# DemianMArin/HMM_Training

Measured on NVIDIA B200. Metric: baum_welch_frames_per_s_per_iter, higher is better.
Workload: dtype f64

## Files before the change

hmm_training_b200/csrc/bw.cu:

```cuda
#include <algorithm>
#include <cstdlib>
#include <functional>
#include <memory>
#include <numeric>

#include "bw_kernels.cuh"
#include "bwltr_kernels.cuh"
#include "viterbi_kernels.cuh"

namespace hmmb {

__global__ void k_load_B(const double *__restrict__ B, int N, int M, double *__restrict__ Bt,
                         int32_t *__restrict__ b_has_zero) {
    const size_t w = blockIdx.y;
    for (int e = blockIdx.x * blockDim.x + threadIdx.x; e < N * M; e += gridDim.x * blockDim.x) {
        const int k = e / N, j = e - k * N;
        const double v = B[(w * N + j) * M + k];
        Bt[w * (size_t)M * N + e] = v > 0.0 ? v : 0.0;
        if (!(v > 0.0) && b_has_zero) b_has_zero[w] = 1;
    }
}
__global__ void k_load_clamped(const double *__restrict__ src, int64_t n, double *__restrict__ dst) {
    for (int64_t e = (int64_t)blockIdx.x * blockDim.x + threadIdx.x; e < n; e += (int64_t)gridDim.x * blockDim.x) {
        const double v = src[e];
// ... 710 lines not shown
        cudaError_t e = cudaMemcpyAsync(&bad, d_bad, sizeof(int), cudaMemcpyDeviceToHost, c.stream);
        if (e == cudaSuccess) e = cudaStreamSynchronize(c.stream);
        if (e != cudaSuccess) rc = cuda_fail(e, "prepare sync", __FILE__, __LINE__);
    }
    dev_free(d_tmp);
    if (rc != HMMB_OK) return rc;
    if (bad) {
        set_error("codeword out of range: some observation is >= M=%d (reference: IndexError)", M);
        return HMMB_ERR_RANGE;
    }
    return HMMB_OK;
}

}

using namespace hmmb;

struct hmmb_bw {
    SeqSet s;
    SeqSet sl;
    bool has_ltr = false;
    bool use_ltr = false;
    uint8_t *d_allfull = nullptr;
    bool check_bad = false;
    std::unique_ptr<PendingPrepare> pend_release;
    void *d_raw = nullptr;
    bool ltr_only = false;
    int raw_idx_bytes = 0;
    uint32_t *d_thinmask = nullptr;
    int32_t *d_thin_new = nullptr;
    int32_t *d_redo = nullptr;
    int32_t *d_redo_in = nullptr;
    int32_t *d_slot_of = nullptr;
    int32_t *act_cur = nullptr;
    int64_t slot_cap = 0, rstride = 0;
    int n_slots = 0;
    int64_t n_thin_total = 0;
    int bpieces = 0, bpieces_issued = 0;
    cudaEvent_t bt_ready[PendingPrepare::MAX_STAGES] = {};
    double *d_ptmp = nullptr;
    std::vector<int64_t> keep_offsets;
    std::vector<int32_t> keep_words;
    SeqSet &cur() { return use_ltr ? sl : s; }
    int W = 0, N = 0, M = 0;
    double *d_pi = nullptr, *d_A = nullptr, *d_Bt = nullptr;
    double *d_spill = nullptr, *d_llseq = nullptr, *d_accum = nullptr, *d_partials = nullptr;
// ... 20 lines not shown
    bool estep_reduced = false;
    bool params_set = false, any_active = true;
};

static double2 *spill4(hmmb_bw *h) { return reinterpret_cast<double2 *>(h->d_spill) + (size_t)BWD4_SPILL_PAD * 64; }

static void bw_drop_pieces(hmmb_bw *h) {
    for (auto &e : h->bt_ready) {
        if (e) event_put(e);
        e = nullptr;
    }
    h->bpieces = h->bpieces_issued = 0;
    dev_free(h->d_ptmp);
    h->d_ptmp = nullptr;
}

static void bw_release(hmmb_bw *h) {
    if (h->d_ptmp && ctx().inited) cudaStreamSynchronize(ctx().copy_stream);
    bw_drop_pieces(h);
    h->pend_release.reset();
    h->s.release();
    h->sl.release();
    dev_free(h->d_allfull);
    dev_free(h->d_raw);
    dev_free(h->d_pi); dev_free(h->d_A); dev_free(h->d_Bt); dev_free(h->d_spill); dev_free(h->d_llseq);
    dev_free(h->d_accum); dev_free(h->d_partials); dev_free(h->d_prev); dev_free(h->d_hist); dev_free(h->d_active);
    dev_free(h->d_iters); dev_free(h->d_any); dev_free(h->d_cta_begin); dev_free(h->d_cta_begin_fine); dev_free(h->d_seq_begin);
    dev_free(h->d_bzero); dev_free(h->d_flag_base); dev_free(h->d_newflags); dev_free(h->d_nexact); dev_free(h->d_exact_scratch);
    dev_free(h->d_thinmask); dev_free(h->d_thin_new); dev_free(h->d_redo); dev_free(h->d_redo_in); dev_free(h->d_slot_of);
}

static int bw_alloc_accum(hmmb_bw *h) {
    dev_free(h->d_accum);
    h->d_accum = nullptr;
    h->accum_n = (int64_t)h->W * h->astride + (int64_t)h->world * h->W * 2 + (int64_t)h->world * h->slot_cap * h->rstride;
    return dev_alloc_t(&h->d_accum, (size_t)h->accum_n);
}

static int bw_set_params_impl(hmmb_bw *h, const double *pi0, const double *A0, const double *B0, bool sync);
static int bw_after_sync(hmmb_bw *h);

static int bw_finish_create(hmmb_bw *h, int64_t R) {
    Ctx &c = ctx();
    SeqSet &s = h->s;
    const int W = h->W, N = h->N, M = h->M;
    h->nacc = (int64_t)N + (int64_t)N * N + (int64_t)M * N;
// ... 22 lines not shown
    TRYF(dev_alloc_t(&h->d_flag_base, (size_t)std::max<int64_t>(R, 1) + FLAG_HDR));
    h->d_flag = h->d_flag_base + FLAG_HDR;
    TRYF(dev_alloc_t(&h->d_newflags, 1));
    TRYF(dev_alloc_t(&h->d_nexact, 1));
    {
        h->exact_stride = (int64_t)std::max(s.tmax_all, 1) * N;
        int64_t warps = std::min<int64_t>((int64_t)c.sm_count * 8, std::max<int64_t>(1, (256LL << 20) / (h->exact_stride * 8)));
        warps = std::min<int64_t>(warps, std::max<int64_t>(1, (R + 31) / 32));
        h->exact_grid = (int)std::max<int64_t>(1, (warps + BW_WARPS - 1) / BW_WARPS);
        TRYF(dev_alloc_t(&h->d_exact_scratch, (size_t)h->exact_grid * BW_WARPS * h->exact_stride));
    }
    TRYF(dev_alloc_t(&h->d_seq_begin, (size_t)W + 1));
    TRYF(h2d_small(h->d_seq_begin, s.seq_begin.data(), (W + 1) * sizeof(int64_t)));
    size_t spill_bytes;
    if (s.special4) {
        spill_bytes = (size_t)(std::max<int64_t>(s.spill_steps, 1) + BWD4_SPILL_PAD) * 64 * sizeof(double2);
        TRYF(dev_alloc_t(&h->d_partials, (size_t)std::max(std::max(s.ncta, s.ncta_fine), 1) * h->pstride));
        TRYF(dev_alloc_t(&h->d_cta_begin, (size_t)W + 1));
        if (s.ncta_fine > 0) {
            TRYF(dev_alloc_t(&h->d_cta_begin_fine, (size_t)W + 1));
            TRYF(h2d_small(h->d_cta_begin_fine, s.cta_begin_fine.data(), (W + 1) * sizeof(int32_t)));
        }
        TRYF(dev_alloc_t(&h->d_allfull, (size_t)std::max<int64_t>(R, 1)));
        TRYF(h2d_small(h->d_cta_begin, s.cta_begin.data(), (W + 1) * sizeof(int32_t)));
    } else {
        spill_bytes = (size_t)std::max<int64_t>(s.frames, 1) * N * sizeof(double);
        if (h->has_ltr) {
            spill_bytes = std::max(spill_bytes, (size_t)std::max<int64_t>(h->sl.spill_steps, 1) * 32 * N * sizeof(double));
            TRYF(dev_alloc_t(&h->d_allfull, (size_t)std::max<int64_t>(R, 1)));
        }
    }
    int rc = dev_alloc((void **)&h->d_spill, spill_bytes);
    if (rc != HMMB_OK) {
        set_error("alpha spill of %.2f GB does not fit in device memory; shard the sequences over more GPUs",
                  spill_bytes / 1e9);
        return HMMB_ERR_OOM;
    }
#undef TRYF
#undef CUDAF
    return HMMB_OK;
}



int hmmb_bw_create(hmmb_bw_t **out, const void *obs, int idx_bytes, int obs_on_device, const int64_t *offsets,
                   const int32_t *word_of_seq, int64_t R, int W, int N, int M) {
// ... 331 lines not shown
    int nw = bidiag ? BWD4_MAX_WARPS : 12;
    auto bytes = [&](int w) { return (size_t)M * rep * 4 * sizeof(double) + (size_t)w * M * 4 * sizeof(double) + (size_t)w * 4 * sizeof(double); };
    const size_t avail = smem_optin > 20 * 1024 ? smem_optin - 20 * 1024 : 0;
    while (nw > 1 && bytes(nw) > avail) --nw;
    *smem = bytes(nw);
    return nw;
}

template <bool BIDIAG, int MT, int REP>
static int launch_special_estep(hmmb_bw *h) {
    Ctx &c = ctx();
    SeqSet &s = h->s;
    if (s.ncta == 0) { s.pend.reset(); return HMMB_OK; }
    const size_t smem_f = (size_t)h->M * 5 * sizeof(double) + (size_t)((h->M + 15) & ~15);
    size_t smem_b = 0;
    const int bwd_threads = 32 * bwd4_warps(h->M, REP, BIDIAG, c.smem_optin, &smem_b);
    HMMB_CUDA(cudaFuncSetAttribute((k_bw_bwd4<BIDIAG, MT, REP>), cudaFuncAttributeMaxDynamicSharedMemorySize, (int)smem_b));
    const CtaWork *stage_work = s.ncta_fine > 0 ? s.d_work_fine : s.d_work;
    const int stage_ncta = s.ncta_fine > 0 ? s.ncta_fine : s.ncta;
    auto launch_range = [&](int c0, int c1) -> int {
        if (c1 <= c0) return HMMB_OK;
        HMMB_LAUNCH("bw_forward", k_bw_fwd4<BIDIAG>, (c1 - c0) * FWD4_SPLIT, BW_THREADS, smem_f, stage_work + c0, s.d_blks, (const uint4 *)s.d_obs,
                    s.d_len, h->d_pi, h->d_A, h->d_Bt, h->M, spill4(h), h->d_llseq, h->act_cur, h->d_flag,
                    h->d_allfull, FWD4_SPLIT, SYM_MASK);
        HMMB_LAUNCH("bw_backward", (k_bw_bwd4<BIDIAG, MT, REP>), c1 - c0, bwd_threads, smem_b, stage_work + c0, s.d_blks, (const uint4 *)s.d_obs,
                    s.d_len, h->d_A, h->d_Bt, h->M, spill4(h), h->d_llseq, h->act_cur, h->d_bzero,
                    h->d_allfull, h->d_partials + (size_t)c0 * h->pstride, h->pstride, h->d_flag, h->d_newflags);
        return HMMB_OK;
    };
    if (s.pend) {
        PendingPrepare &p = *s.pend;
        int bdone = 0, cdone = 0;
        cudaStream_t main_stream = c.stream;
        const bool side = p.nstage > 2;
        struct Restore { Ctx &c; cudaStream_t s; ~Restore() { c.stream = s; } } restore{c, main_stream};
        if (side) {
            cudaEvent_t fork = event_get();
            HMMB_CUDA(cudaEventRecord(fork, main_stream));
            for (auto st : c.stage_stream) HMMB_CUDA(cudaStreamWaitEvent(st, fork, 0));
            event_put(fork);
        }
        for (int j = 0; j < p.nstage; ++j) {
            if (side) c.stream = c.stage_stream[j & 1];
            HMMB_CUDA(cudaStreamWaitEvent(c.stream, p.up->ev[p.ev_index[j]], 0));
            HMMB_TRY(launch_repack_range(s, p.up->d_raw, p.idx_bytes, bdone, p.blk_end[j], s.d_bad));
            HMMB_TRY(launch_range(cdone, p.cta_end[j]));
            bdone = p.blk_end[j];
            cdone = p.cta_end[j];
        }
        c.stream = main_stream;
        if (side) {
            for (auto st : c.stage_stream) {
                cudaEvent_t join = event_get();
                HMMB_CUDA(cudaEventRecord(join, st));
                HMMB_CUDA(cudaStreamWaitEvent(main_stream, join, 0));
                event_put(join);
            }
        }
        h->check_bad = true;
        h->pend_release = std::move(s.pend);
        HMMB_TRY((launch_exact<uint16_t, true>(h)));
        HMMB_LAUNCH("bw_exact", k_bw_llstat_fix, stage_ncta, BW_THREADS, 0, stage_work, s.d_blks, h->d_llseq, h->act_cur,
                    h->d_flag, h->d_partials, h->pstride, h->M);
        h->estep_fine = s.ncta_fine > 0;
        return HMMB_OK;
    }
    h->estep_fine = false;
    HMMB_LAUNCH("bw_forward", k_bw_fwd4<BIDIAG>, (s.ncta_fwd ? s.ncta_fwd : s.ncta) * FWD4_SPLIT, BW_THREADS, smem_f,
                s.ncta_fwd ? s.d_work_fwd : s.d_work, s.d_blks, (const uint4 *)s.d_obs,
                s.d_len, h->d_pi, h->d_A, h->d_Bt, h->M, spill4(h), h->d_llseq, h->act_cur, h->d_flag,
                h->d_allfull, FWD4_SPLIT, SYM_MASK);
    HMMB_TRY((launch_exact<uint16_t, true>(h)));
    HMMB_LAUNCH("bw_backward", (k_bw_bwd4<BIDIAG, MT, REP>), s.ncta, bwd_threads, smem_b, s.d_work, s.d_blks, (const uint4 *)s.d_obs,
                s.d_len, h->d_A, h->d_Bt, h->M, spill4(h), h->d_llseq, h->act_cur, h->d_bzero,
                h->d_allfull, h->d_partials, h->pstride, h->d_flag, h->d_newflags);
    return HMMB_OK;
}

template <int NS>
static int launch_ltr_estep(hmmb_bw *h) {
    SeqSet &s = h->sl;
    if (s.ncta == 0) return HMMB_OK;
    const int M = h->M;
    const size_t smem_f = (size_t)M * NS * 8 + (size_t)M * 8 + (size_t)M * 2;
    const size_t smem_b = (size_t)M * NS * 8 + (size_t)LTR_WARPS * 32 * Ltr<NS>::ROWB + (size_t)2 * NS * 8 +
                          (size_t)LTR_WARPS * 2 * NS * 8;
    HMMB_CUDA(cudaFuncSetAttribute(k_bw_fwdL<NS>, cudaFuncAttributeMaxDynamicSharedMemorySize, (int)smem_f));
    HMMB_CUDA(cudaFuncSetAttribute(k_bw_bwdL<NS>, cudaFuncAttributeMaxDynamicSharedMemorySize, (int)smem_b));
    if (s.pend) {
        Ctx &c = ctx();
        PendingPrepare &p = *s.pend;
        int bdone = 0, cdone = 0;
        cudaStream_t main_stream = c.stream;
        const bool side = p.nstage > 2;
        struct Restore { Ctx &c; cudaStream_t s; ~Restore() { c.stream = s; } } restore{c, main_stream};
        if (side) {
            cudaEvent_t fork = event_get();
            HMMB_CUDA(cudaEventRecord(fork, main_stream));
// ... 618 lines not shown
```

hmm_training_b200/csrc/bw4_kernels.cuh:

```cuda
#pragma once

#include <type_traits>

#include "hmm_device.cuh"

namespace hmmb {

constexpr int BW_THREADS = 128;
constexpr int BW_WARPS = BW_THREADS / 32;
constexpr int SPC4 = 8;
constexpr unsigned SYM_MASK = 0x7ffu;
constexpr int SYM_BITS = 11;
constexpr int BW4_MAX_M = 512;
constexpr int BWD4_MAX_WARPS = 16;
constexpr int FWD4_SPLIT = 4;
constexpr int BWD4_REP = 8;

constexpr int REPACK_WARPS = 8;
__device__ __forceinline__ unsigned lanes_with_my_bit(unsigned sym, int bit) {
    int mine;
    asm("bfe.s32 %0, %1, %2, 1;" : "=r"(mine) : "r"(sym), "r"(bit));
    const unsigned set = __ballot_sync(0xffffffffu, mine != 0);
    return ~(set ^ (unsigned)mine);
}
// ... 92 lines not shown
        for (int j = 0; j < 4; ++j) row[i] |= (__ldg(Aw + i * 4 + j) > 0.0) ? (1u << j) : 0u;
    }
    Masks4 mk;
    mk.lutF = mk.lutB = 0ull;
    for (unsigned m = 0; m < 16; ++m) {
        unsigned f = 0u, b = 0u;
#pragma unroll
        for (int i = 0; i < 4; ++i) {
            if ((m >> i) & 1u) f |= row[i];
            if (row[i] & m) b |= 1u << i;
        }
        mk.lutF |= (unsigned long long)f << (m * 4u);
        mk.lutB |= (unsigned long long)b << (m * 4u);
    }
    mk.pmask = 0u;
    if (piw) {
#pragma unroll
        for (int j = 0; j < 4; ++j) mk.pmask |= (__ldg(piw + j) > 0.0) ? (1u << j) : 0u;
    }
    return mk;
}
__device__ __forceinline__ double tiny_if(unsigned m, int j) { return __hiloint2double(0, (int)((m >> j) & 1u)); }

template <bool BIDIAG, bool SPILL, bool VECB = true, int REP = 1>
__device__ __forceinline__ double fwd4_run(int T, int tmax, const uint4 *__restrict__ op,
                                           const double2 *__restrict__ sB01, const double2 *__restrict__ sB23,
                                           const double *__restrict__ sBmax,
                                           const unsigned char *__restrict__ sBmask, const double *a,
                                           const double (&p)[4], double rmax, const Masks4 &mk,
                                           double2 *__restrict__ sp, bool &allfull, int slot = 0,
                                           unsigned symmask = SYM_MASK) {
    using S16 = Sym<uint16_t>;
    double al0 = 0.0, al1 = 0.0, al2 = 0.0, al3 = 0.0;
    double e0 = 0.0, e1 = 0.0, e2 = 0.0, e3 = 0.0;
    long long esum = 0;
    unsigned m = 0u;
    bool stop = false;
    bool allf = true;
    double ll = neg_inf();
    const double tiny = tiny_pos();
    const int nch = (tmax + SPC4 - 1) / SPC4;
    uint4 wnext = nch > 0 ? __ldg(op) : make_uint4(0, 0, 0, 0);
    for (int c = 0; c < nch; ++c) {
        uint4 w = wnext;
        if (c + 1 < nch) wnext = __ldg(op + (size_t)(c + 1) * 32);
#pragma unroll 2
        for (int s = 0; s < SPC4; ++s) {
            const int t = c * SPC4 + s;
            const unsigned sym = S16::pop_front(w) & symmask;
            if (t < T && !stop) {
                const double2 b01 = sB01[sym * REP + slot], b23 = sB23[sym * REP + slot];
                const unsigned r = (t == 0) ? mk.pmask : lut4(mk.lutF, m);
                m = r & (unsigned)sBmask[sym];
                double n0, n1, n2, n3, at0, at1, at2, at3;
                if (m == 0xFu && t > 0) {
                    if (BIDIAG) {
                        n0 = fma(al0, a[0], tiny);
                        n1 = fma(al1, a[1], fma(al0, a[4], tiny));
                        n2 = fma(al2, a[2], fma(al1, a[5], tiny));
                        n3 = fma(al3, a[3], fma(al2, a[6], tiny));
                    } else {
                        n0 = fma(al3, a[12], fma(al2, a[8], fma(al1, a[4], fma(al0, a[0], tiny))));
                        n1 = fma(al3, a[13], fma(al2, a[9], fma(al1, a[5], fma(al0, a[1], tiny))));
                        n2 = fma(al3, a[14], fma(al2, a[10], fma(al1, a[6], fma(al0, a[2], tiny))));
                        n3 = fma(al3, a[15], fma(al2, a[11], fma(al1, a[7], fma(al0, a[3], tiny))));
                    }
                    at0 = fma(n0, b01.x, tiny); at1 = fma(n1, b01.y, tiny);
                    at2 = fma(n2, b23.x, tiny); at3 = fma(n3, b23.y, tiny);
                } else if (m == 0u) {
                    stop = true;
                    n0 = n1 = n2 = n3 = at0 = at1 = at2 = at3 = 0.0;
                } else {
                    allf = allf && (m == 0xFu);
                    const double r0 = tiny_if(r, 0), r1 = tiny_if(r, 1), r2 = tiny_if(r, 2), r3 = tiny_if(r, 3);
                    if (t == 0) {
                        n0 = p[0]; n1 = p[1]; n2 = p[2]; n3 = p[3];
                    } else {
                        n0 = fma(al3, a_at<BIDIAG>(a, 3, 0), fma(al2, a_at<BIDIAG>(a, 2, 0), fma(al1, a_at<BIDIAG>(a, 1, 0), fma(al0, a_at<BIDIAG>(a, 0, 0), r0))));
                        n1 = fma(al3, a_at<BIDIAG>(a, 3, 1), fma(al2, a_at<BIDIAG>(a, 2, 1), fma(al1, a_at<BIDIAG>(a, 1, 1), fma(al0, a_at<BIDIAG>(a, 0, 1), r1))));
                        n2 = fma(al3, a_at<BIDIAG>(a, 3, 2), fma(al2, a_at<BIDIAG>(a, 2, 2), fma(al1, a_at<BIDIAG>(a, 1, 2), fma(al0, a_at<BIDIAG>(a, 0, 2), r2))));
                        n3 = fma(al3, a_at<BIDIAG>(a, 3, 3), fma(al2, a_at<BIDIAG>(a, 2, 3), fma(al1, a_at<BIDIAG>(a, 1, 3), fma(al0, a_at<BIDIAG>(a, 0, 3), r3))));
                    }
                    at0 = fma(n0, b01.x, tiny_if(m, 0)); at1 = fma(n1, b01.y, tiny_if(m, 1));
                    at2 = fma(n2, b23.x, tiny_if(m, 2)); at3 = fma(n3, b23.y, tiny_if(m, 3));
                }
                double ssum = (at0 + at1) + (at2 + at3);
                if (!stop && !(ssum >= TINY_STEP)) {
                    double o[4];
                    int Ex;
                    const int code = exact_products4(n0, n1, n2, n3, b01.x, b01.y, b23.x, b23.y, o, &Ex);
                    if (code == 0) {
                        stop = true;
                    } else if ((code == 2 && t > 0) || ((e0 + e1) + (e2 + e3)) > 0.0) {
                        stop = true;
                        ll = nan_mark();
                    } else {
                        esum += Ex;
                        at0 = o[0]; at1 = o[1]; at2 = o[2]; at3 = o[3];
                        ssum = (at0 + at1) + (at2 + at3);
                    }
                    allf = false;
                }
                if (!stop) {
                    const double sc = pow2_rescale(ssum, esum);
                    allf = allf && (__double2hiint(sc) >= 0x3ff00000);
                    al0 = at0 * sc; al1 = at1 * sc; al2 = at2 * sc; al3 = at3 * sc;
                    if (!VECB) {
                        e0 = fma(e0, rmax * sBmax[sym], 4.0 * ERR_UNIT) * sc;
                    } else {
                    double f0 = 0.0, f1 = 0.0, f2 = 0.0, f3 = 0.0;
                    if (t > 0) {
                        if (BIDIAG) {
                            f0 = e0 * a[0];
                            f1 = fma(e1, a[1], e0 * a[4]);
                            f2 = fma(e2, a[2], e1 * a[5]);
                            f3 = fma(e3, a[3], e2 * a[6]);
                        } else {
                            f0 = fma(e3, a[12], fma(e2, a[8], fma(e1, a[4], e0 * a[0])));
                            f1 = fma(e3, a[13], fma(e2, a[9], fma(e1, a[5], e0 * a[1])));
                            f2 = fma(e3, a[14], fma(e2, a[10], fma(e1, a[6], e0 * a[2])));
                            f3 = fma(e3, a[15], fma(e2, a[11], fma(e1, a[7], e0 * a[3])));
                        }
                    }
                    e0 = fma(f0, b01.x, ERR_UNIT) * sc;
                    e1 = fma(f1, b01.y, ERR_UNIT) * sc;
                    e2 = fma(f2, b23.x, ERR_UNIT) * sc;
                    e3 = fma(f3, b23.y, ERR_UNIT) * sc;
                    }
                    if (!(((e0 + e1) + (e2 + e3)) <= ERR_LIMIT)) {
                        stop = true;
                        ll = nan_mark();
                    }
                    if (t == T - 1 && !stop) ll = log((al0 + al1) + (al2 + al3)) + (double)esum * LN2;
                }
                if (SPILL && !stop) {
                    __stcs(sp + (size_t)t * 64, make_double2(al0, al1));
                    __stcs(sp + (size_t)t * 64 + 32, make_double2(al2, al3));
                }
            }
        }
    }
    allfull = allf && !stop;
    return ll;
}

template <bool BIDIAG, int REP>
__device__ __forceinline__ double score4_lean_run(int T, int tmax, const uint4 *__restrict__ op,
                                                  const double2 *__restrict__ b01row, const double2 *__restrict__ b23row,
                                                  const double *a, const double (&p)[4], const Masks4 &mk, int tstar,
                                                  bool &bad_out) {
    using S16 = Sym<uint16_t>;
    double al0 = 0.0, al1 = 0.0, al2 = 0.0, al3 = 0.0;
    int esum = 0;
    bool bad = false;
    unsigned m = 0u;
    auto step = [&](auto masked, int t, unsigned sym) {
        constexpr bool MASKED = decltype(masked)::value;
        const double2 b01 = b01row[sym * REP], b23 = b23row[sym * REP];
        double n0, n1, n2, n3;
        if (MASKED && t == 0) {
            n0 = p[0]; n1 = p[1]; n2 = p[2]; n3 = p[3];
        } else {
            matvec_fwd<BIDIAG>(a, al0, al1, al2, al3, n0, n1, n2, n3);
        }
        const double at0 = n0 * b01.x, at1 = n1 * b01.y, at2 = n2 * b23.x, at3 = n3 * b23.y;
// ... 81 lines not shown
    }
    load_Api4<BIDIAG>(pi, A, w, a, p, rmax, mk);
}

template <bool BIDIAG>
__device__ __forceinline__ void load_A4(const double *__restrict__ Aw, double *a) {
    if (BIDIAG) {
#pragma unroll
        for (int i = 0; i < 4; ++i) a[i] = __ldg(Aw + i * 5);
#pragma unroll
        for (int i = 0; i < 3; ++i) a[4 + i] = __ldg(Aw + i * 5 + 1);
    } else {
#pragma unroll
        for (int q = 0; q < 16; ++q) a[q] = __ldg(Aw + q);
    }
}

constexpr int FWD4_MIN_CTAS = 4;
template <bool BIDIAG>
__global__ void __launch_bounds__(BW_THREADS, FWD4_MIN_CTAS)
k_bw_fwd4(const CtaWork *__restrict__ work, const Blk *__restrict__ blks, const uint4 *__restrict__ obs_blk,
          const int32_t *__restrict__ len_sorted, const double *__restrict__ pi, const double *__restrict__ A,
          const double *__restrict__ Bt, int M, double2 *__restrict__ spill, double *__restrict__ ll_seq,
          const int32_t *__restrict__ active, uint8_t *__restrict__ flag, uint8_t *__restrict__ allfull, int split,
          unsigned symmask) {
    extern __shared__ double sB[];
    double *sBmax = sB + (size_t)M * 4;
    unsigned char *sBmask = reinterpret_cast<unsigned char *>(sBmax + M);
    CtaWork cw = work[blockIdx.x / split];
    if (!active[cw.word]) return;
    {
        const int nb = cw.blk_end - cw.blk_begin, part = blockIdx.x % split;
        const int lo = cw.blk_begin + (int)((int64_t)nb * part / split);
        cw.blk_end = cw.blk_begin + (int)((int64_t)nb * (part + 1) / split);
        cw.blk_begin = lo;
        if (cw.blk_begin >= cw.blk_end) return;
    }
    const int tid = threadIdx.x, lane = tid & 31, warp = tid >> 5;
    double a[BIDIAG ? 7 : 16], p[4], rmax;
    Masks4 mk;
    load_model4<BIDIAG>(pi, A, Bt, cw.word, M, sB, sBmax, sBmask, a, p, rmax, mk);
    __syncthreads();
    for (int b = cw.blk_begin + warp; b < cw.blk_end; b += BW_WARPS) {
        const Blk bk = blks[b];
        int T = lane < bk.nseq ? len_sorted[bk.first + lane] : 0;
        if (T > 0 && flag[bk.first + lane]) T = 0;
        bool af = false;
        const double ll = fwd4_run<BIDIAG, true>(T, bk.tmax, obs_blk + bk.obs_base + lane, reinterpret_cast<const double2 *>(sB),
                                                 reinterpret_cast<const double2 *>(sB) + M, sBmax, sBmask, a, p, rmax,
                                                 mk, spill + bk.spill_base * 64 + lane, af, 0, symmask);
        if (T > 0) {
            ll_seq[bk.first + lane] = ll;
            allfull[bk.first + lane] = af ? 1 : 0;
            if (ll != ll) raise_flag(flag, bk.first + lane);
        }
    }
}

__device__ __forceinline__ unsigned smem_u32(const void *p) { return (unsigned)__cvta_generic_to_shared(p); }
__device__ __forceinline__ unsigned hold32(unsigned x) { return __shfl_sync(0xffffffffu, x, threadIdx.x & 31); }
__device__ __forceinline__ double2 lds128_ro(unsigned addr) {
    double2 v;
    asm("ld.shared.v2.f64 {%0, %1}, [%2];" : "=d"(v.x), "=d"(v.y) : "r"(addr));
    return v;
}
__device__ __forceinline__ double2 lds128(unsigned addr) {
    double2 v;
    asm volatile("ld.shared.v2.f64 {%0, %1}, [%2];" : "=d"(v.x), "=d"(v.y) : "r"(addr) : "memory");
    return v;
}
__device__ __forceinline__ void sts128(unsigned addr, double2 v) {
    asm volatile("st.shared.v2.f64 [%0], {%1, %2};" ::"r"(addr), "d"(v.x), "d"(v.y) : "memory");
}
// ... 206 lines not shown
    if (tid == 0) {
        out[0] = m;
        out[1] = ((sRed[0][1] + sRed[1][1]) + sRed[2][1]) + sRed[3][1];
    }
    (void)nwarps;
}

__global__ void __launch_bounds__(BW_THREADS)
k_bw_llstat_fix(const CtaWork *__restrict__ work, const Blk *__restrict__ blks, const double *__restrict__ ll_seq,
                const int32_t *__restrict__ active, const uint8_t *__restrict__ flag, double *__restrict__ partials,
                int64_t pstride, int M) {
    if (!any_flag_raised(flag)) return;
    __shared__ double sRed[BW_WARPS][20];
    const CtaWork cw = work[blockIdx.x];
    if (!active[cw.word]) return;
    cta_ll_stat(blks, cw, ll_seq, sRed, partials + (size_t)blockIdx.x * pstride + 20 + (size_t)M * 4);
}

template <bool BIDIAG, int MT, int REP>
__global__ void __launch_bounds__(BIDIAG ? BWD4_MAX_WARPS * 32 : 384, 1)
k_bw_bwd4(const CtaWork *__restrict__ work, const Blk *__restrict__ blks, const uint4 *__restrict__ obs_blk,
          const int32_t *__restrict__ len_sorted, const double *__restrict__ A, const double *__restrict__ Bt, int M_rt,
          const double2 *__restrict__ spill, const double *__restrict__ ll_seq, const int32_t *__restrict__ active,
          const int32_t *__restrict__ b_has_zero, const uint8_t *__restrict__ allfull, double *__restrict__ partials,
          int64_t pstride, uint8_t *__restrict__ flag, int32_t *__restrict__ new_flags) {
    using S16 = Sym<uint16_t>;
    const int M = MT ? MT : M_rt;
    const int nthreads = blockDim.x, nwarps = nthreads >> 5;
    extern __shared__ double smem[];
    double *sB = smem;
    double *sCnt = smem + (size_t)M * REP * 4;
    double *sPi = sCnt + (size_t)M * 4 * nwarps;
    __shared__ double sRed[BWD4_MAX_WARPS][20];
    __shared__ unsigned sSeen;
    __shared__ uint4 sW[2][BWD4_MAX_WARPS * 32];

    const CtaWork cw = work[blockIdx.x];
    double *part = partials + (size_t)blockIdx.x * pstride;
    const int tid = threadIdx.x, lane = tid & 31, warp = tid >> 5;
    if (!active[cw.word]) return;
    {
        const double2 *src = reinterpret_cast<const double2 *>(Bt + (size_t)cw.word * M * 4);
        double2 *dst01 = reinterpret_cast<double2 *>(sB), *dst23 = dst01 + (size_t)M * REP;
        for (int e = tid; e < M * REP; e += nthreads) {
            const int sym = e / REP;
            dst01[e] = __ldg(src + 2 * sym);
            dst23[e] = __ldg(src + 2 * sym + 1);
        }
        for (int e = tid; e < M * 4 * nwarps + nwarps * 4; e += nthreads) sCnt[e] = 0.0;
        if (tid == 0) sSeen = 0u;
    }
    double a[BIDIAG ? 7 : 16];
    load_A4<BIDIAG>(A + (size_t)cw.word * 16, a);
    const Masks4 mk = make_masks4(A + (size_t)cw.word * 16, nullptr);
    const bool lean_ok = (b_has_zero[cw.word] == 0) && (lut4(mk.lutB, 0xFu) == 0xFu);
    const double tiny = tiny_pos();
    __syncthreads();

    double2 *cntw01 = reinterpret_cast<double2 *>(sCnt + (size_t)warp * M * 4);
    const double2 *sB01 = reinterpret_cast<const double2 *>(sB) + (lane & (REP - 1)), *sB23 = sB01 + (size_t)M * REP;
    double *mypi = sPi + (size_t)warp * 4;
    const unsigned bbase = hold32(smem_u32(sB01)), cbase = hold32(smem_u32(cntw01));
    const unsigned B23_OFF = (unsigned)M * REP * 16u, CNT23_OFF = (unsigned)M * 16u;
    Bwd4State<BIDIAG> st;
#pragma unroll
    for (int q = 0; q < (BIDIAG ? 7 : 16); ++q) st.X[q] = 0.0;
    st.seenX = 0u;

    for (int b = cw.blk_begin + warp; b < cw.blk_end; b += nwarps) {
        const Blk bk = blks[b];
        int T = 0;
        bool apos = false;
        if (lane < bk.nseq) {
            T = len_sorted[bk.first + lane];
            if (!(ll_seq[bk.first + lane] > neg_inf())) T = 0;
            if (flag[bk.first + lane]) T = 0;
            apos = allfull[bk.first + lane] != 0;
        }
        st.v0 = st.v1 = st.v2 = st.v3 = 0.0;
        st.imprecise = false;
        st.vpos = false;
        st.rref = 1.0;
        const uint4 *op = obs_blk + bk.obs_base + lane;
        const double2 *sp = spill + bk.spill_base * 64 + lane;
        const int nch = (bk.tmax + SPC4 - 1) / SPC4;
        double2 P0_01 = make_double2(0.0, 0.0), P0_23 = P0_01, P1_01 = P0_01, P1_23 = P0_01;
        {
            const int r1 = nch * SPC4, r0 = max(r1 - BWD_L2_PREFETCH, 0);
            const char *base = reinterpret_cast<const char *>(sp - lane) + (size_t)r0 * 1024;
            for (int l = lane; l < (r1 - r0) * 8; l += 32) prefetch_l2(base + (size_t)l * 128);
            const int ta = bk.tmax - 1;
            if (ta < T) {
                const double2 x01 = __ldcs(sp + (size_t)ta * 64), x23 = __ldcs(sp + (size_t)ta * 64 + 32);
                if (ta & 1) { P1_01 = x01; P1_23 = x23; }
                else        { P0_01 = x01; P0_23 = x23; }
            }
        }
        int wbuf = 0;
        cp_async16(&sW[0][tid], op + (size_t)(nch - 1) * 32);
        cp_async_commit();

#define HMMB_BWD_STEP(T_, C_, O_, SP_, PACKED_)                                                                     \
    {                                                                                                               \
        const int t = (T_);                                                                                         \
        const double2 *spt = (SP_);          \
        const unsigned packed = (PACKED_);                                                                          \
        if (t < bk.tmax) {                                                                        \
            const unsigned sym = packed & SYM_MASK;                                                                 \
            const bool act = t < T;                                                                                 \
            const double al0 = P##C_##_01.x, al1 = P##C_##_01.y, al2 = P##C_##_23.x, al3 = P##C_##_23.y;            \
             \
             \
             \
             \
            P##O_##_01 = __ldcs(spt - 64);                                                                          \
            P##O_##_23 = __ldcs(spt - 64 + 32);                                                                     \
            const unsigned brow = bbase + sym * (unsigned)(REP * 16);                                               \
            const unsigned crow = cbase + sym * 16u;                                                                \
            const int rank = (int)(packed >> SYM_BITS);                                                             \
            double g0 = undef_f64(), g1 = undef_f64(), g2 = undef_f64(), g3 = undef_f64();                          \
            if (act) {                                                                                              \
                bool done = false;                                                                                  \
                if (lean_ok && st.vpos) {              \
                        \
                       \
                        \
                    double q0, q1, q2, q3;                                                                          \
                    if (BIDIAG) {                                                                                   \
                        q0 = fma(a[4], st.v1, fma(a[0], st.v0, tiny));                                              \
                        q1 = fma(a[5], st.v2, fma(a[1], st.v1, tiny));                                              \
                        q2 = fma(a[6], st.v3, fma(a[2], st.v2, tiny));                                              \
                        q3 = fma(a[3], st.v3, tiny);                                                                \
                    } else {                                                                                        \
                        q0 = fma(a[3], st.v3, fma(a[2], st.v2, fma(a[1], st.v1, fma(a[0], st.v0, tiny))));          \
                        q1 = fma(a[7], st.v3, fma(a[6], st.v2, fma(a[5], st.v1, fma(a[4], st.v0, tiny))));          \
                        q2 = fma(a[11], st.v3, fma(a[10], st.v2, fma(a[9], st.v1, fma(a[8], st.v0, tiny))));        \
                        q3 = fma(a[15], st.v3, fma(a[14], st.v2, fma(a[13], st.v1, fma(a[12], st.v0, tiny))));      \
                    }                                                                                               \
                    const double qs = (q0 + q1) + (q2 + q3);                                                        \
                    const double c0 = al0 * q0, c1 = al1 * q1, c2 = al2 * q2, c3 = al3 * q3;                        \
                    const double norm = (c0 + c1) + (c2 + c3);                                                      \
                    const double r = recip_from_ref(norm, st.rref);                \
// ... 1 lines not shown
                    const unsigned lo2 = min((unsigned)__double2hiint(norm), (unsigned)__double2hiint(qs));         \
                    if ((lo2 >= LEAN_MIN_HI) & norm_consistent(norm, r) && (apos || all_pos4(al0, al1, al2, al3))) {\
                                 \
                        g0 = fma(c0, r, tiny); g1 = fma(c1, r, tiny); g2 = fma(c2, r, tiny); g3 = fma(c3, r, tiny); \
                        const double u0 = al0 * r, u1 = al1 * r, u2 = al2 * r, u3 = al3 * r;                        \
                        if (BIDIAG) {                                                                               \
                            st.X[0] = fma(u0, st.v0, st.X[0]); st.X[1] = fma(u1, st.v1, st.X[1]);                   \
                            st.X[2] = fma(u2, st.v2, st.X[2]); st.X[3] = fma(u3, st.v3, st.X[3]);                   \
                            st.X[4] = fma(u0, st.v1, st.X[4]); st.X[5] = fma(u1, st.v2, st.X[5]);                   \
                            st.X[6] = fma(u2, st.v3, st.X[6]);                                                      \
                        } else {                                                                                    \
                            st.X[0] = fma(u0, st.v0, st.X[0]);   st.X[1] = fma(u0, st.v1, st.X[1]);                 \
                            st.X[2] = fma(u0, st.v2, st.X[2]);   st.X[3] = fma(u0, st.v3, st.X[3]);                 \
                            st.X[4] = fma(u1, st.v0, st.X[4]);   st.X[5] = fma(u1, st.v1, st.X[5]);                 \
                            st.X[6] = fma(u1, st.v2, st.X[6]);   st.X[7] = fma(u1, st.v3, st.X[7]);                 \
                            st.X[8] = fma(u2, st.v0, st.X[8]);   st.X[9] = fma(u2, st.v1, st.X[9]);                 \
                            st.X[10] = fma(u2, st.v2, st.X[10]); st.X[11] = fma(u2, st.v3, st.X[11]);               \
                            st.X[12] = fma(u3, st.v0, st.X[12]); st.X[13] = fma(u3, st.v1, st.X[13]);               \
                            st.X[14] = fma(u3, st.v2, st.X[14]); st.X[15] = fma(u3, st.v3, st.X[15]);               \
                        }                                                                                           \
                        st.seenX = 0xffffu;                                \
                        const double sc = pow2_rescale_noacc(qs);                                                   \
                        const double h0 = q0 * sc, h1 = q1 * sc, h2 = q2 * sc, h3 = q3 * sc;        \
                        const double2 b01 = lds128_ro(brow), b23 = lds128_ro(brow + B23_OFF);                       \
                        st.v0 = fma(b01.x, h0, tiny); st.v1 = fma(b01.y, h1, tiny);                                 \
                        st.v2 = fma(b23.x, h2, tiny); st.v3 = fma(b23.y, h3, tiny);                                 \
                        const double vs = (st.v0 + st.v1) + (st.v2 + st.v3);                                        \
                        if ((unsigned)__double2hiint(vs) < LEAN_MIN_HI) {      \
                            double vv[4];                                                                           \
                             \
                            if (bwd4_v_slow(zero_to_tiny(h0), zero_to_tiny(h1), zero_to_tiny(h2), zero_to_tiny(h3), b01.x, b01.y,       \
                                            b23.x, b23.y, vv)) st.imprecise = true;   \
                            st.v0 = vv[0]; st.v1 = vv[1]; st.v2 = vv[2]; st.v3 = vv[3];                             \
                            st.vpos = all_pos4(vv[0], vv[1], vv[2], vv[3]);                                         \
                        }                                                                                           \
                        done = true;                                                                                \
                    }                                                                                               \
                }                                                                                                   \
                if (!done) {                                                                                        \
                    if (t == T - 1) {                                                                               \
                        \
                        \
                        \
                        const double n0 = (al0 + al1) + (al2 + al3);   \
                        const double r0 = 1.0 / n0;                                                                 \
                        st.rref = r0;                                                                               \
                        g0 = fma(al0, r0, pos_to_tiny(al0)); g1 = fma(al1, r0, pos_to_tiny(al1));                   \
                        g2 = fma(al2, r0, pos_to_tiny(al2)); g3 = fma(al3, r0, pos_to_tiny(al3));                   \
                        const double2 b01 = lds128_ro(brow), b23 = lds128_ro(brow + B23_OFF);                       \
                        st.v0 = b01.x; st.v1 = b01.y; st.v2 = b23.x; st.v3 = b23.y;                                 \
                        st.vpos = all_pos4(b01.x, b01.y, b23.x, b23.y);                                             \
                    } else {                                                                                        \
                              \
                             \
                        Bwd4State<BIDIAG> tmp = st;                                                                 \
                        double g[4];                                                                                \
                        bwd4_step_slow<BIDIAG>(tmp, a, sB01, sB23, sym * REP, false, al0, al1, al2, al3, g);        \
                        st = tmp;                                                                                   \
                        g0 = g[0]; g1 = g[1]; g2 = g[2]; g3 = g[3];                                                 \
                    }                                                                                               \
                }                                                                                                   \
            }                                                                                                       \
            if (t == 0) {  \
                const int am = act ? -1 : 0;          \
                double p0 = __hiloint2double(__double2hiint(g0) & am, __double2loint(g0) & am);                     \
                double p1 = __hiloint2double(__double2hiint(g1) & am, __double2loint(g1) & am);                     \
                double p2 = __hiloint2double(__double2hiint(g2) & am, __double2loint(g2) & am);                     \
                double p3 = __hiloint2double(__double2hiint(g3) & am, __double2loint(g3) & am);                     \
                _Pragma("unroll") for (int o = 16; o > 0; o >>= 1) {                                                \
                    p0 += __shfl_xor_sync(0xffffffffu, p0, o); p1 += __shfl_xor_sync(0xffffffffu, p1, o);           \
                    p2 += __shfl_xor_sync(0xffffffffu, p2, o); p3 += __shfl_xor_sync(0xffffffffu, p3, o);           \
                }                                                                                                   \
                if (lane == 0) { mypi[0] += p0; mypi[1] += p1; mypi[2] += p2; mypi[3] += p3; }                      \
            }                                                                                                       \
                            \
            cnt_update4(crow, CNT23_OFF, act, rank, g0, g1, g2, g3);                                                \
        }                                                                                                           \
    }

        const double2 *spp = sp + (size_t)(nch * SPC4 - 2) * 64;
        for (int c = nch - 1; c >= 0; --c) {
            cp_async_wait_all();
            uint4 w = sW[wbuf][tid];
            wbuf ^= 1;
            if (c > 0) {
                cp_async16(&sW[wbuf][tid], op + (size_t)(c - 1) * 32);
                cp_async_commit();
            }
#pragma unroll 1
            for (int pr = SPC4 / 2 - 1; pr >= 0; --pr) {
                if (c * SPC4 + 2 * pr >= BWD_L2_PREFETCH && lane < 16)
                    prefetch_l2(reinterpret_cast<const char *>(spp) - BWD_L2_PREFETCH * 1024 + lane * (128 - 16));
                const unsigned p1 = S16::pop_back(w);
                HMMB_BWD_STEP(c * SPC4 + 2 * pr + 1, 1, 0, spp + 64, p1)
                const unsigned p0 = S16::pop_back(w);
                HMMB_BWD_STEP(c * SPC4 + 2 * pr, 0, 1, spp, p0)
                spp -= 2 * 64;
            }
        }
#undef HMMB_BWD_STEP
        if (st.imprecise) {
            raise_flag(flag, bk.first + lane);
            atomicAdd(new_flags, 1);
        }
    }

    double Xf[16];
    if (BIDIAG) {
#pragma unroll
        for (int q = 0; q < 16; ++q) Xf[q] = 0.0;
        Xf[0] = st.X[0]; Xf[5] = st.X[1]; Xf[10] = st.X[2]; Xf[15] = st.X[3];
        Xf[1] = st.X[4]; Xf[6] = st.X[5]; Xf[11] = st.X[6];
    } else {
#pragma unroll
        for (int q = 0; q < 16; ++q) Xf[q] = st.X[q];
    }
#pragma unroll
    for (int q = 0; q < 16; ++q) {
        double v = Xf[q];
// ... 36 lines not shown
```

Baseline: 66.07 billion.

## Skip odd-step alpha spills in a plain window and recompute them in backward

The forward pass now tracks a per-sequence window of 'plain' steps (all states alive, rescale factor at least one). Inside that window it stores only even-step alphas to the spill buffer and records the window bounds in a new per-sequence array. The backward pass reloads the even-step alpha and recomputes the odd-step alpha from it with one forward transition and rescale, and only reads stored odd steps outside the window. L2 prefetching is cut to match. This roughly halves spill write and read traffic in exchange for extra FMAs in the backward pass, more register pressure, and a risk of small numeric differences from the recomputation.

```diff
diff --git a/hmm_training_b200/csrc/bw.cu b/hmm_training_b200/csrc/bw.cu
--- a/hmm_training_b200/csrc/bw.cu
+++ b/hmm_training_b200/csrc/bw.cu
@@ -756,6 +756,7 @@
     bool has_ltr = false;
     bool use_ltr = false;
     uint8_t *d_allfull = nullptr;
+    unsigned *d_rwin4 = nullptr;
     bool check_bad = false;
     std::unique_ptr<PendingPrepare> pend_release;
     void *d_raw = nullptr;
@@ -822,6 +823,7 @@
     h->s.release();
     h->sl.release();
     dev_free(h->d_allfull);
+    dev_free(h->d_rwin4);
     dev_free(h->d_raw);
     dev_free(h->d_pi); dev_free(h->d_A); dev_free(h->d_Bt); dev_free(h->d_spill); dev_free(h->d_llseq);
     dev_free(h->d_accum); dev_free(h->d_partials); dev_free(h->d_prev); dev_free(h->d_hist); dev_free(h->d_active);
@@ -890,6 +892,7 @@
             TRYF(h2d_small(h->d_cta_begin_fine, s.cta_begin_fine.data(), (W + 1) * sizeof(int32_t)));
         }
         TRYF(dev_alloc_t(&h->d_allfull, (size_t)std::max<int64_t>(R, 1)));
+        TRYF(dev_alloc_t(&h->d_rwin4, (size_t)std::max<int64_t>(R, 1)));
         TRYF(h2d_small(h->d_cta_begin, s.cta_begin.data(), (W + 1) * sizeof(int32_t)));
     } else {
         spill_bytes = (size_t)std::max<int64_t>(s.frames, 1) * N * sizeof(double);
@@ -1267,10 +1270,10 @@
         if (c1 <= c0) return HMMB_OK;
         HMMB_LAUNCH("bw_forward", k_bw_fwd4<BIDIAG>, (c1 - c0) * FWD4_SPLIT, BW_THREADS, smem_f, stage_work + c0, s.d_blks, (const uint4 *)s.d_obs,
                     s.d_len, h->d_pi, h->d_A, h->d_Bt, h->M, spill4(h), h->d_llseq, h->act_cur, h->d_flag,
-                    h->d_allfull, FWD4_SPLIT, SYM_MASK);
+                    h->d_allfull, h->d_rwin4, FWD4_SPLIT, SYM_MASK);
         HMMB_LAUNCH("bw_backward", (k_bw_bwd4<BIDIAG, MT, REP>), c1 - c0, bwd_threads, smem_b, stage_work + c0, s.d_blks, (const uint4 *)s.d_obs,
                     s.d_len, h->d_A, h->d_Bt, h->M, spill4(h), h->d_llseq, h->act_cur, h->d_bzero,
-                    h->d_allfull, h->d_partials + (size_t)c0 * h->pstride, h->pstride, h->d_flag, h->d_newflags);
+                    h->d_allfull, h->d_rwin4, h->d_partials + (size_t)c0 * h->pstride, h->pstride, h->d_flag, h->d_newflags);
         return HMMB_OK;
     };
     if (s.pend) {
@@ -1314,11 +1317,11 @@
     HMMB_LAUNCH("bw_forward", k_bw_fwd4<BIDIAG>, (s.ncta_fwd ? s.ncta_fwd : s.ncta) * FWD4_SPLIT, BW_THREADS, smem_f,
                 s.ncta_fwd ? s.d_work_fwd : s.d_work, s.d_blks, (const uint4 *)s.d_obs,
                 s.d_len, h->d_pi, h->d_A, h->d_Bt, h->M, spill4(h), h->d_llseq, h->act_cur, h->d_flag,
-                h->d_allfull, FWD4_SPLIT, SYM_MASK);
+                h->d_allfull, h->d_rwin4, FWD4_SPLIT, SYM_MASK);
     HMMB_TRY((launch_exact<uint16_t, true>(h)));
     HMMB_LAUNCH("bw_backward", (k_bw_bwd4<BIDIAG, MT, REP>), s.ncta, bwd_threads, smem_b, s.d_work, s.d_blks, (const uint4 *)s.d_obs,
                 s.d_len, h->d_A, h->d_Bt, h->M, spill4(h), h->d_llseq, h->act_cur, h->d_bzero,
-                h->d_allfull, h->d_partials, h->pstride, h->d_flag, h->d_newflags);
+                h->d_allfull, h->d_rwin4, h->d_partials, h->pstride, h->d_flag, h->d_newflags);
     return HMMB_OK;
 }
 
diff --git a/hmm_training_b200/csrc/bw4_kernels.cuh b/hmm_training_b200/csrc/bw4_kernels.cuh
--- a/hmm_training_b200/csrc/bw4_kernels.cuh
+++ b/hmm_training_b200/csrc/bw4_kernels.cuh
@@ -138,6 +138,55 @@
 }
 __device__ __forceinline__ double tiny_if(unsigned m, int j) { return __hiloint2double(0, (int)((m >> j) & 1u)); }
 
+template <bool BIDIAG>
+__device__ __forceinline__ double fwd4_alive_products(const double *a, double al0, double al1, double al2, double al3,
+                                                      double2 b01, double2 b23, double &n0, double &n1, double &n2,
+                                                      double &n3, double &at0, double &at1, double &at2, double &at3) {
+    const double tiny = tiny_pos();
+    if (BIDIAG) {
+        n0 = fma(al0, a[0], tiny);
+        n1 = fma(al1, a[1], fma(al0, a[4], tiny));
+        n2 = fma(al2, a[2], fma(al1, a[5], tiny));
+        n3 = fma(al3, a[3], fma(al2, a[6], tiny));
+    } else {
+        n0 = fma(al3, a[12], fma(al2, a[8], fma(al1, a[4], fma(al0, a[0], tiny))));
+        n1 = fma(al3, a[13], fma(al2, a[9], fma(al1, a[5], fma(al0, a[1], tiny))));
+        n2 = fma(al3, a[14], fma(al2, a[10], fma(al1, a[6], fma(al0, a[2], tiny))));
+        n3 = fma(al3, a[15], fma(al2, a[11], fma(al1, a[7], fma(al0, a[3], tiny))));
+    }
+    at0 = fma(n0, b01.x, tiny); at1 = fma(n1, b01.y, tiny);
+    at2 = fma(n2, b23.x, tiny); at3 = fma(n3, b23.y, tiny);
+    return (at0 + at1) + (at2 + at3);
+}
+template <bool BIDIAG>
+__device__ __forceinline__ double fwd4_products(const double *a, const double *p, bool first, unsigned r, unsigned m,
+                                                double al0, double al1, double al2, double al3, double2 b01, double2 b23,
+                                                double &n0, double &n1, double &n2, double &n3, double &at0,
+                                                double &at1, double &at2, double &at3) {
+    if (m == 0xFu && !first) {
+        return fwd4_alive_products<BIDIAG>(a, al0, al1, al2, al3, b01, b23, n0, n1, n2, n3, at0, at1, at2, at3);
+    } else {
+        const double r0 = tiny_if(r, 0), r1 = tiny_if(r, 1), r2 = tiny_if(r, 2), r3 = tiny_if(r, 3);
+        if (first) {
+            n0 = p[0]; n1 = p[1]; n2 = p[2]; n3 = p[3];
+        } else {
+            n0 = fma(al3, a_at<BIDIAG>(a, 3, 0), fma(al2, a_at<BIDIAG>(a, 2, 0), fma(al1, a_at<BIDIAG>(a, 1, 0), fma(al0, a_at<BIDIAG>(a, 0, 0), r0))));
+            n1 = fma(al3, a_at<BIDIAG>(a, 3, 1), fma(al2, a_at<BIDIAG>(a, 2, 1), fma(al1, a_at<BIDIAG>(a, 1, 1), fma(al0, a_at<BIDIAG>(a, 0, 1), r1))));
+            n2 = fma(al3, a_at<BIDIAG>(a, 3, 2), fma(al2, a_at<BIDIAG>(a, 2, 2), fma(al1, a_at<BIDIAG>(a, 1, 2), fma(al0, a_at<BIDIAG>(a, 0, 2), r2))));
+            n3 = fma(al3, a_at<BIDIAG>(a, 3, 3), fma(al2, a_at<BIDIAG>(a, 2, 3), fma(al1, a_at<BIDIAG>(a, 1, 3), fma(al0, a_at<BIDIAG>(a, 0, 3), r3))));
+        }
+        at0 = fma(n0, b01.x, tiny_if(m, 0)); at1 = fma(n1, b01.y, tiny_if(m, 1));
+        at2 = fma(n2, b23.x, tiny_if(m, 2)); at3 = fma(n3, b23.y, tiny_if(m, 3));
+    }
+    return (at0 + at1) + (at2 + at3);
+}
+__device__ __forceinline__ void fwd4_rescale(double sc, double at0, double at1, double at2, double at3, double &al0,
+                                             double &al1, double &al2, double &al3) {
+    al0 = at0 * sc; al1 = at1 * sc; al2 = at2 * sc; al3 = at3 * sc;
+}
+
+constexpr int WIN_LO_END = 256;
+constexpr int WIN_HI_END = 1 << 24;
 template <bool BIDIAG, bool SPILL, bool VECB = true, int REP = 1>
 __device__ __forceinline__ double fwd4_run(int T, int tmax, const uint4 *__restrict__ op,
                                            const double2 *__restrict__ sB01, const double2 *__restrict__ sB23,
@@ -145,7 +194,7 @@
                                            const unsigned char *__restrict__ sBmask, const double *a,
                                            const double (&p)[4], double rmax, const Masks4 &mk,
                                            double2 *__restrict__ sp, bool &allfull, int slot = 0,
-                                           unsigned symmask = SYM_MASK) {
+                                           unsigned symmask = SYM_MASK, unsigned *win_out = nullptr) {
     using S16 = Sym<uint16_t>;
     double al0 = 0.0, al1 = 0.0, al2 = 0.0, al3 = 0.0;
     double e0 = 0.0, e1 = 0.0, e2 = 0.0, e3 = 0.0;
@@ -153,8 +202,8 @@
     unsigned m = 0u;
     bool stop = false;
     bool allf = true;
+    bool started = false, inwin = false;
     double ll = neg_inf();
-    const double tiny = tiny_pos();
     const int nch = (tmax + SPC4 - 1) / SPC4;
     uint4 wnext = nch > 0 ? __ldg(op) : make_uint4(0, 0, 0, 0);
     for (int c = 0; c < nch; ++c) {
@@ -168,39 +217,17 @@
                 const double2 b01 = sB01[sym * REP + slot], b23 = sB23[sym * REP + slot];
                 const unsigned r = (t == 0) ? mk.pmask : lut4(mk.lutF, m);
                 m = r & (unsigned)sBmask[sym];
-                double n0, n1, n2, n3, at0, at1, at2, at3;
-                if (m == 0xFu && t > 0) {
-                    if (BIDIAG) {
-                        n0 = fma(al0, a[0], tiny);
-                        n1 = fma(al1, a[1], fma(al0, a[4], tiny));
-                        n2 = fma(al2, a[2], fma(al1, a[5], tiny));
-                        n3 = fma(al3, a[3], fma(al2, a[6], tiny));
-                    } else {
-                        n0 = fma(al3, a[12], fma(al2, a[8], fma(al1, a[4], fma(al0, a[0], tiny))));
-                        n1 = fma(al3, a[13], fma(al2, a[9], fma(al1, a[5], fma(al0, a[1], tiny))));
-                        n2 = fma(al3, a[14], fma(al2, a[10], fma(al1, a[6], fma(al0, a[2], tiny))));
-                        n3 = fma(al3, a[15], fma(al2, a[11], fma(al1, a[7], fma(al0, a[3], tiny))));
-                    }
-                    at0 = fma(n0, b01.x, tiny); at1 = fma(n1, b01.y, tiny);
-                    at2 = fma(n2, b23.x, tiny); at3 = fma(n3, b23.y, tiny);
-                } else if (m == 0u) {
+                double n0, n1, n2, n3, at0, at1, at2, at3, ssum;
+                bool plain = false;
+                if (m == 0u) {
                     stop = true;
-                    n0 = n1 = n2 = n3 = at0 = at1 = at2 = at3 = 0.0;
+                    n0 = n1 = n2 = n3 = at0 = at1 = at2 = at3 = ssum = 0.0;
                 } else {
                     allf = allf && (m == 0xFu);
-                    const double r0 = tiny_if(r, 0), r1 = tiny_if(r, 1), r2 = tiny_if(r, 2), r3 = tiny_if(r, 3);
-                    if (t == 0) {
-                        n0 = p[0]; n1 = p[1]; n2 = p[2]; n3 = p[3];
-                    } else {
-                        n0 = fma(al3, a_at<BIDIAG>(a, 3, 0), fma(al2, a_at<BIDIAG>(a, 2, 0), fma(al1, a_at<BIDIAG>(a, 1, 0), fma(al0, a_at<BIDIAG>(a, 0, 0), r0))));
-                        n1 = fma(al3, a_at<BIDIAG>(a, 3, 1), fma(al2, a_at<BIDIAG>(a, 2, 1), fma(al1, a_at<BIDIAG>(a, 1, 1), fma(al0, a_at<BIDIAG>(a, 0, 1), r1))));
-                        n2 = fma(al3, a_at<BIDIAG>(a, 3, 2), fma(al2, a_at<BIDIAG>(a, 2, 2), fma(al1, a_at<BIDIAG>(a, 1, 2), fma(al0, a_at<BIDIAG>(a, 0, 2), r2))));
-                        n3 = fma(al3, a_at<BIDIAG>(a, 3, 3), fma(al2, a_at<BIDIAG>(a, 2, 3), fma(al1, a_at<BIDIAG>(a, 1, 3), fma(al0, a_at<BIDIAG>(a, 0, 3), r3))));
-                    }
-                    at0 = fma(n0, b01.x, tiny_if(m, 0)); at1 = fma(n1, b01.y, tiny_if(m, 1));
-                    at2 = fma(n2, b23.x, tiny_if(m, 2)); at3 = fma(n3, b23.y, tiny_if(m, 3));
+                    plain = (m == 0xFu) && t > 0;
+                    ssum = fwd4_products<BIDIAG>(a, p, t == 0, r, m, al0, al1, al2, al3, b01, b23, n0, n1, n2, n3, at0,
+                                                 at1, at2, at3);
                 }
-                double ssum = (at0 + at1) + (at2 + at3);
                 if (!stop && !(ssum >= TINY_STEP)) {
                     double o[4];
                     int Ex;
@@ -216,11 +243,14 @@
                         ssum = (at0 + at1) + (at2 + at3);
                     }
                     allf = false;
+                    plain = false;
                 }
                 if (!stop) {
                     const double sc = pow2_rescale(ssum, esum);
-                    allf = allf && (__double2hiint(sc) >= 0x3ff00000);
-                    al0 = at0 * sc; al1 = at1 * sc; al2 = at2 * sc; al3 = at3 * sc;
+                    const bool sc_ge1 = __double2hiint(sc) >= 0x3ff00000;
+                    allf = allf && sc_ge1;
+                    plain = plain && sc_ge1;
+                    fwd4_rescale(sc, at0, at1, at2, at3, al0, al1, al2, al3);
                     if (!VECB) {
                         e0 = fma(e0, rmax * sBmax[sym], 4.0 * ERR_UNIT) * sc;
                     } else {
@@ -249,7 +279,14 @@
                     }
                     if (t == T - 1 && !stop) ll = log((al0 + al1) + (al2 + al3)) + (double)esum * LN2;
                 }
-                if (SPILL && !stop) {
+                if (SPILL) {
+                    const bool in = plain && (inwin ? t < WIN_HI_END : (!started && t < WIN_LO_END));
+                    if (in && !started) *win_out = (unsigned)t;
+                    if (inwin && !in) *win_out |= (unsigned)t << 8;
+                    started = started || plain;
+                    inwin = in;
+                }
+                if (SPILL && !stop && (!(t & 1) || !inwin)) {
                     __stcs(sp + (size_t)t * 64, make_double2(al0, al1));
                     __stcs(sp + (size_t)t * 64 + 32, make_double2(al2, al3));
                 }
@@ -257,6 +294,10 @@
         }
     }
     allfull = allf && !stop;
+    if (SPILL && T > 0) {
+        if (!started) *win_out = 0u;
+        else if (inwin) *win_out |= (unsigned)T << 8;
+    }
     return ll;
 }
 
@@ -384,8 +425,8 @@
 k_bw_fwd4(const CtaWork *__restrict__ work, const Blk *__restrict__ blks, const uint4 *__restrict__ obs_blk,
           const int32_t *__restrict__ len_sorted, const double *__restrict__ pi, const double *__restrict__ A,
           const double *__restrict__ Bt, int M, double2 *__restrict__ spill, double *__restrict__ ll_seq,
-          const int32_t *__restrict__ active, uint8_t *__restrict__ flag, uint8_t *__restrict__ allfull, int split,
-          unsigned symmask) {
+          const int32_t *__restrict__ active, uint8_t *__restrict__ flag, uint8_t *__restrict__ allfull,
+          unsigned *__restrict__ rwin, int split, unsigned symmask) {
     extern __shared__ double sB[];
     double *sBmax = sB + (size_t)M * 4;
     unsigned char *sBmask = reinterpret_cast<unsigned char *>(sBmax + M);
@@ -410,7 +451,7 @@
         bool af = false;
         const double ll = fwd4_run<BIDIAG, true>(T, bk.tmax, obs_blk + bk.obs_base + lane, reinterpret_cast<const double2 *>(sB),
                                                  reinterpret_cast<const double2 *>(sB) + M, sBmax, sBmask, a, p, rmax,
-                                                 mk, spill + bk.spill_base * 64 + lane, af, 0, symmask);
+                                                 mk, spill + bk.spill_base * 64 + lane, af, 0, symmask, rwin + bk.first + lane);
         if (T > 0) {
             ll_seq[bk.first + lane] = ll;
             allfull[bk.first + lane] = af ? 1 : 0;
@@ -663,8 +704,8 @@
 k_bw_bwd4(const CtaWork *__restrict__ work, const Blk *__restrict__ blks, const uint4 *__restrict__ obs_blk,
           const int32_t *__restrict__ len_sorted, const double *__restrict__ A, const double *__restrict__ Bt, int M_rt,
           const double2 *__restrict__ spill, const double *__restrict__ ll_seq, const int32_t *__restrict__ active,
-          const int32_t *__restrict__ b_has_zero, const uint8_t *__restrict__ allfull, double *__restrict__ partials,
-          int64_t pstride, uint8_t *__restrict__ flag, int32_t *__restrict__ new_flags) {
+          const int32_t *__restrict__ b_has_zero, const uint8_t *__restrict__ allfull, const unsigned *__restrict__ rwin,
+          double *__restrict__ partials, int64_t pstride, uint8_t *__restrict__ flag, int32_t *__restrict__ new_flags) {
     using S16 = Sym<uint16_t>;
     const int M = MT ? MT : M_rt;
     const int nthreads = blockDim.x, nwarps = nthreads >> 5;
@@ -711,12 +752,14 @@
     for (int b = cw.blk_begin + warp; b < cw.blk_end; b += nwarps) {
         const Blk bk = blks[b];
         int T = 0;
+        unsigned win = 0u;
         bool apos = false;
         if (lane < bk.nseq) {
             T = len_sorted[bk.first + lane];
             if (!(ll_seq[bk.first + lane] > neg_inf())) T = 0;
             if (flag[bk.first + lane]) T = 0;
             apos = allfull[bk.first + lane] != 0;
+            win = rwin[bk.first + lane];
         }
         st.v0 = st.v1 = st.v2 = st.v3 = 0.0;
         st.imprecise = false;
@@ -725,23 +768,22 @@
         const uint4 *op = obs_blk + bk.obs_base + lane;
         const double2 *sp = spill + bk.spill_base * 64 + lane;
         const int nch = (bk.tmax + SPC4 - 1) / SPC4;
-        double2 P0_01 = make_double2(0.0, 0.0), P0_23 = P0_01, P1_01 = P0_01, P1_23 = P0_01;
+        double2 P0_01 = make_double2(0.0, 0.0), P0_23 = P0_01;
         {
             const int r1 = nch * SPC4, r0 = max(r1 - BWD_L2_PREFETCH, 0);
             const char *base = reinterpret_cast<const char *>(sp - lane) + (size_t)r0 * 1024;
-            for (int l = lane; l < (r1 - r0) * 8; l += 32) prefetch_l2(base + (size_t)l * 128);
-            const int ta = bk.tmax - 1;
-            if (ta < T) {
-                const double2 x01 = __ldcs(sp + (size_t)ta * 64), x23 = __ldcs(sp + (size_t)ta * 64 + 32);
-                if (ta & 1) { P1_01 = x01; P1_23 = x23; }
-                else        { P0_01 = x01; P0_23 = x23; }
+            for (int l = lane; l < (r1 - r0) / 2 * 8; l += 32) prefetch_l2(base + (size_t)(l >> 3) * 2048 + (l & 7) * 128);
+            const int te = (bk.tmax - 1) & ~1;
+            if (te < T) {
+                P0_01 = __ldcs(sp + (size_t)te * 64);
+                P0_23 = __ldcs(sp + (size_t)te * 64 + 32);
             }
         }
         int wbuf = 0;
         cp_async16(&sW[0][tid], op + (size_t)(nch - 1) * 32);
         cp_async_commit();
 
-#define HMMB_BWD_STEP(T_, C_, O_, SP_, PACKED_)                                                                     \
+#define HMMB_BWD_STEP(T_, ODD_, SP_, PACKED_)                                                                       \
     {                                                                                                               \
         const int t = (T_);                                                                                         \
         const double2 *spt = (SP_);          \
@@ -749,16 +791,38 @@
         if (t < bk.tmax) {                                                                        \
             const unsigned sym = packed & SYM_MASK;                                                                 \
             const bool act = t < T;                                                                                 \
-            const double al0 = P##C_##_01.x, al1 = P##C_##_01.y, al2 = P##C_##_23.x, al3 = P##C_##_23.y;            \
-             \
-             \
-             \
-             \
-            P##O_##_01 = __ldcs(spt - 64);                                                                          \
-            P##O_##_23 = __ldcs(spt - 64 + 32);                                                                     \
             const unsigned brow = bbase + sym * (unsigned)(REP * 16);                                               \
             const unsigned crow = cbase + sym * 16u;                                                                \
             const int rank = (int)(packed >> SYM_BITS);                                                             \
+            double al0 = undef_f64(), al1 = undef_f64(), al2 = undef_f64(), al3 = undef_f64();                      \
+            double2 b01 = make_double2(undef_f64(), undef_f64()), b23 = b01;                                        \
+            if (!(ODD_)) {                                                                                          \
+                al0 = P0_01.x; al1 = P0_01.y; al2 = P0_23.x; al3 = P0_23.y;                                         \
+                \
+                \
+                \
+                \
+                P0_01 = __ldcs(spt - 128);                                                                          \
+                P0_23 = __ldcs(spt - 128 + 32);                                                                     \
+                if (act) { b01 = lds128_ro(brow); b23 = lds128_ro(brow + B23_OFF); }                                \
+            } else {                                                                                                \
+                          \
+                const bool stored = act && (t < (int)(win & 0xFFu) || t >= (int)(win >> 8));                       \
+                if (__any_sync(0xffffffffu, stored) && stored) {                                                    \
+                    const double2 x01 = __ldcs(spt), x23 = __ldcs(spt + 32);                                        \
+                    al0 = x01.x; al1 = x01.y; al2 = x23.x; al3 = x23.y;                                             \
+                }                                                                                                   \
+                if (act) {                                                                                          \
+                                           \
+                    b01 = lds128_ro(brow); b23 = lds128_ro(brow + B23_OFF);                                         \
+                    if (!stored) {                                                                                  \
+                        double n0, n1, n2, n3, at0, at1, at2, at3;                                                  \
+                        const double ssum = fwd4_alive_products<BIDIAG>(a, P0_01.x, P0_01.y, P0_23.x, P0_23.y, b01, \
+                                                                        b23, n0, n1, n2, n3, at0, at1, at2, at3);   \
+                        fwd4_rescale(pow2_rescale_noacc(ssum), at0, at1, at2, at3, al0, al1, al2, al3);             \
+                    }                                                                                               \
+                }                                                                                                   \
+            }                                                                                                       \
             double g0 = undef_f64(), g1 = undef_f64(), g2 = undef_f64(), g3 = undef_f64();                          \
             if (act) {                                                                                              \
                 bool done = false;                                                                                  \
@@ -806,7 +870,6 @@
                         st.seenX = 0xffffu;                                \
                         const double sc = pow2_rescale_noacc(qs);                                                   \
                         const double h0 = q0 * sc, h1 = q1 * sc, h2 = q2 * sc, h3 = q3 * sc;        \
-                        const double2 b01 = lds128_ro(brow), b23 = lds128_ro(brow + B23_OFF);                       \
                         st.v0 = fma(b01.x, h0, tiny); st.v1 = fma(b01.y, h1, tiny);                                 \
                         st.v2 = fma(b23.x, h2, tiny); st.v3 = fma(b23.y, h3, tiny);                                 \
                         const double vs = (st.v0 + st.v1) + (st.v2 + st.v3);                                        \
@@ -831,7 +894,6 @@
                         st.rref = r0;                                                                               \
                         g0 = fma(al0, r0, pos_to_tiny(al0)); g1 = fma(al1, r0, pos_to_tiny(al1));                   \
                         g2 = fma(al2, r0, pos_to_tiny(al2)); g3 = fma(al3, r0, pos_to_tiny(al3));                   \
-                        const double2 b01 = lds128_ro(brow), b23 = lds128_ro(brow + B23_OFF);                       \
                         st.v0 = b01.x; st.v1 = b01.y; st.v2 = b23.x; st.v3 = b23.y;                                 \
                         st.vpos = all_pos4(b01.x, b01.y, b23.x, b23.y);                                             \
                     } else {                                                                                        \
@@ -873,12 +935,12 @@
             }
 #pragma unroll 1
             for (int pr = SPC4 / 2 - 1; pr >= 0; --pr) {
-                if (c * SPC4 + 2 * pr >= BWD_L2_PREFETCH && lane < 16)
+                if (c * SPC4 + 2 * pr >= BWD_L2_PREFETCH && lane < 8)
                     prefetch_l2(reinterpret_cast<const char *>(spp) - BWD_L2_PREFETCH * 1024 + lane * (128 - 16));
                 const unsigned p1 = S16::pop_back(w);
-                HMMB_BWD_STEP(c * SPC4 + 2 * pr + 1, 1, 0, spp + 64, p1)
+                HMMB_BWD_STEP(c * SPC4 + 2 * pr + 1, 1, spp + 64, p1)
                 const unsigned p0 = S16::pop_back(w);
-                HMMB_BWD_STEP(c * SPC4 + 2 * pr, 0, 1, spp, p0)
+                HMMB_BWD_STEP(c * SPC4 + 2 * pr, 0, spp, p0)
                 spp -= 2 * 64;
             }
         }
```

Measured after the change: 63.06 billion (median of 6 runs). 4.6% lower.
